# kr-colab/locator

Hardware: AMD Instinct MI355X
Metric: training samples/sec on 1000x100k-SNP matrix (higher is better)
Workload: dtype f32; 1 GPU; synthetic 1000 ind x 100000 SNPs uint8 (BASELINE.json configs[2]), single model fit per GPU, batch 32, 810 train / 90 validation; width=256, nlayers=10, graph=True, chained_steps=True, epochs_in_flight=2, replicates_per_gpu=1, replicates=single model, full=False

## Files before the change

locator_amd/_abi.py:

```python
import ctypes as C
import os
import re
from typing import NamedTuple

HEADER = os.path.join(os.path.dirname(os.path.dirname(os.path.abspath(__file__))), "include", "locator_hip.h")
_EXTENSION_TABLE = (
    ("ext", "locator_hip_query.h", None),
    ("region", "locator_hip_regions.h", "LOC_REGION_"),
    ("neighbor", "locator_hip_neighbors.h", "LOC_IBS_"),
    ("pca", "locator_hip_pca.h", "LOC_PCA_"),
    ("ld", "locator_hip_ld.h", "LOC_LD_"),
    ("spa", "locator_hip_spa.h", "LOC_SPA_"),
    ("admix", "locator_hip_admix.h", "LOC_ADMIX_"),
    ("localpca", "locator_hip_localpca.h", "LOC_LOCALPCA_"),
    ("paint", "locator_hip_paint.h", "LOC_PAINT_"),
    ("ibd", "locator_hip_ibd.h", "LOC_IBD_"),
    ("impute", "locator_hip_impute.h", "LOC_IMPUTE_"),
)

_SCALARS = {"int": C.c_int, "int32_t": C.c_int32, "uint32_t": C.c_uint32, "int64_t": C.c_int64, "uint64_t": C.c_uint64,
            "float": C.c_float, "double": C.c_double}
_POINTEES = ("void", "char", "int8_t", "uint8_t")
_BY_REFERENCE = ("loc_dims", "loc_layout", "loc_net", "loc_tuning")

_FIRST = re.compile(r"(?:const\s+)?(\w+)\s*((?:\*\s*)*)(\w+)$")
_NEXT = re.compile(r"((?:\*\s*)*)(\w+)$")
_DEFINE = re.compile(r"^[ \t]*#[ \t]*define[ \t]+(LOC_\w+)[ \t]+(\S.*?)[ \t]*$", re.M)
_STRUCT = re.compile(r"typedef\s+struct\s+(\w+)\s*\{(.*?)\}\s*\1\s*;", re.S)
_PROTO = re.compile(r"(.*?)\b(loc_\w+)\s*\((.*)\)$", re.S)


def _ctype(base, stars, name, structs, arg):
# ... 59 lines not shown
if not os.path.exists(HEADER):
    raise FileNotFoundError(f"{HEADER} not found: locator_amd runs in-tree and derives its ctypes binding from "
                            "include/locator_hip.h (the same relative path locator_amd/csrc compiles against).")
with open(HEADER) as _f:
    CONSTANTS, STRUCTS, PROTOTYPES = parse(_f.read())
globals().update(CONSTANTS)


class Extension(NamedTuple):
    header: str
    constants: dict
    prototypes: dict


EXTENSIONS = {}
ALL_PROTOTYPES = dict(PROTOTYPES)
_declared = set(CONSTANTS) | set(PROTOTYPES)
for _tag, _name, _prefix in _EXTENSION_TABLE:
    _path = os.path.join(os.path.dirname(HEADER), _name)
    if not os.path.exists(_path):
        raise FileNotFoundError(f"{_path} not found: it declares entry points added after include/locator_hip.h")
    with open(_path) as _f:
        _consts, _structs, _protos = parse(_f.read())
    _again = sorted(_declared & (set(_consts) | set(_protos)))
    _foreign = sorted(k for k, v in _consts.items() if _prefix is None or not k.startswith(_prefix) or not isinstance(v, int))
    if _structs or _again or _foreign or _tag in EXTENSIONS:
        raise ValueError(f"{_path} may declare new functions " + ("only" if _prefix is None else f"and {_prefix}* integer constants only")
                         + "".join(f"; {what}: {', '.join(names)}" for what, names in (("declared before", _again), ("not such a constant", _foreign))
                                   if names))
    _declared |= set(_consts) | set(_protos)
    EXTENSIONS[_tag] = Extension(_path, _consts, _protos)
    ALL_PROTOTYPES.update(_protos)
    globals().update(_consts)
```

locator_amd/csrc/l1_kernels.hip:

```cpp
#include <stdlib.h>

#include <type_traits>

#include "common.h"

#define LP 36

__global__ __launch_bounds__(128) void bn_batch_stats_kernel(
    const uint8_t* __restrict__ X, int64_t pitch, const int32_t* __restrict__ rows, int n_b, int K, int Kp,
    const float* __restrict__ gamma, const float* __restrict__ beta, float* __restrict__ mov_mean,
    float* __restrict__ mov_var, float* __restrict__ out4) {
    const int k0 = (blockIdx.x * blockDim.x + threadIdx.x) * 4;
    if (k0 >= Kp) return;
    int s[4] = {0, 0, 0, 0}, ss[4] = {0, 0, 0, 0};
#pragma unroll 8
    for (int b = 0; b < n_b; ++b) {
        uint32_t v = *reinterpret_cast<const uint32_t*>(X + (int64_t)rows[b] * pitch + k0);
#pragma unroll
        for (int c = 0; c < 4; ++c) {
            int x = (v >> (8 * c)) & 255;
            s[c] += x;
            ss[c] += x * x;
        }
    }
// ... 9 lines not shown
            o_sc[c] = scale;
            o_sh[c] = beta[k] - mean * scale;
            o_mu[c] = mean;
            o_rs[c] = rstd;
            mov_mean[k] = mov_mean[k] * BN_MOMENTUM + mean * (1.0f - BN_MOMENTUM);
            mov_var[k] = mov_var[k] * BN_MOMENTUM + var * (1.0f - BN_MOMENTUM);
        }
    }
    *reinterpret_cast<f32x4*>(out4 + k0) = o_sc;
    *reinterpret_cast<f32x4*>(out4 + Kp + k0) = o_sh;
    *reinterpret_cast<f32x4*>(out4 + 2 * (int64_t)Kp + k0) = o_mu;
    *reinterpret_cast<f32x4*>(out4 + 3 * (int64_t)Kp + k0) = o_rs;
}

template <bool UNIT>
__global__ __launch_bounds__(128) void bn_epoch_stats_kernel(const uint8_t* __restrict__ X, int64_t pitch,
                                                             const int32_t* __restrict__ rows_all, int batch,
                                                             int n_last, int n_steps, int K, int Kp,
                                                             float* __restrict__ stats_ep, float var_add) {
    const int k0 = (blockIdx.x * blockDim.x + threadIdx.x) * 4;
    const int step = blockIdx.y;
    if (k0 >= Kp) return;
    const int n_b = step == n_steps - 1 ? n_last : batch;
    const int32_t* rows = rows_all + (int64_t)step * batch;
    int s[4] = {0, 0, 0, 0}, ss[4] = {0, 0, 0, 0};
#pragma unroll 8
    for (int b = 0; b < n_b; ++b) {
        uint32_t v = *reinterpret_cast<const uint32_t*>(X + (int64_t)rows[b] * pitch + k0);
#pragma unroll
        for (int c = 0; c < 4; ++c) {
            int x = (v >> (8 * c)) & 255;
            s[c] += x;
            ss[c] += x * x;
        }
    }
    f32x4 mu = {0, 0, 0, 0}, var = {0, 0, 0, 0};
#pragma unroll
    for (int c = 0; c < 4; ++c) {
        if (k0 + c < K) {
            mu[c] = (float)s[c] / (float)n_b;
            var[c] = (float)((int64_t)n_b * ss[c] - (int64_t)s[c] * s[c]) / ((float)n_b * (float)n_b);
            if constexpr (UNIT) var[c] += var_add;
        }
    }
    float* o = stats_ep + (int64_t)step * 2 * Kp;
    *reinterpret_cast<f32x4*>(o + k0) = mu;
    *reinterpret_cast<f32x4*>(o + Kp + k0) = var;
}

__global__ void bn_epoch_finish_kernel(int K, int Kp, int n_steps, const float* __restrict__ stats_ep,
                                       const float* __restrict__ gamma, const float* __restrict__ beta,
                                       float* __restrict__ mov_mean, float* __restrict__ mov_var,
                                       float* __restrict__ bn4) {
    const int k = blockIdx.x * blockDim.x + threadIdx.x;
    if (k >= Kp) return;
    float scale = 0.f, shift = 0.f, mean0 = 0.f, rstd0 = 0.f;
    if (k < K) {
        float mm = mov_mean[k], mv = mov_var[k];
        for (int j = 0; j < n_steps; ++j) {
            const float mu = stats_ep[(int64_t)j * 2 * Kp + k], var = stats_ep[(int64_t)j * 2 * Kp + Kp + k];
            mm = mm * BN_MOMENTUM + mu * (1.0f - BN_MOMENTUM);
            mv = mv * BN_MOMENTUM + var * (1.0f - BN_MOMENTUM);
        }
        mov_mean[k] = mm;
        mov_var[k] = mv;
        mean0 = stats_ep[k];
        rstd0 = 1.0f / sqrtf(stats_ep[Kp + k] + BN_EPS);
        scale = gamma[k] * rstd0;
        shift = beta[k] - mean0 * scale;
    }
    if (bn4 == nullptr) return;
    bn4[k] = scale;
    bn4[Kp + k] = shift;
    bn4[2 * (int64_t)Kp + k] = mean0;
    bn4[3 * (int64_t)Kp + k] = rstd0;
}

__global__ void bn_infer_scale_shift_kernel(int K, int Kp, const float* __restrict__ gamma,
                                            const float* __restrict__ beta, const float* __restrict__ mov_mean,
                                            const float* __restrict__ mov_var, float* __restrict__ out4) {
    int k = blockIdx.x * blockDim.x + threadIdx.x;
    if (k >= Kp) return;
    float scale = 0.f, shift = 0.f, mean = 0.f, rstd = 0.f;
    if (k < K) {
        mean = mov_mean[k];
        rstd = 1.0f / sqrtf(mov_var[k] + BN_EPS);
        scale = gamma[k] * rstd;
        shift = beta[k] - mean * scale;
    }
    out4[k] = scale;
    out4[Kp + k] = shift;
    out4[2 * (int64_t)Kp + k] = mean;
    out4[3 * (int64_t)Kp + k] = rstd;
}

template <int NHT>
__global__ __launch_bounds__(512) void l1_fwd_partial_kernel(const uint8_t* __restrict__ X, int64_t pitch,
                                                             const int32_t* __restrict__ rows, int n_b, int Kp,
                                                             const float* __restrict__ ss4,
                                                             const float* __restrict__ w1s,
                                                             float* __restrict__ partial,
                                                             const uint8_t* __restrict__ in_mask, float in_ks) {
    constexpr int Hp = NHT * 32;
// ... 620 lines not shown
    if (k >= K) return;
    const float alpha = adam_alpha(alpha_tab, alpha_tab_len, lr, t_base, t_off);
    gamma_beta_adam_body(k, Kp, gbs, gamma, beta, m_gamma, v_gamma, m_beta, v_beta, alpha, next_stats, bn4);
}

extern "C" int loc_bn_batch_stats(const uint8_t* X, int64_t x_pitch, const int32_t* rows, int n_b, int K, int Kp,
                                  const float* gamma, const float* beta, float* mov_mean, float* mov_var,
                                  float* out4, void* stream) {
    if (n_b < 1 || n_b > LOC_ROWS) { loc_set_error("loc_bn_batch_stats: n_b=%d out of 1..32", n_b); return -1; }
    hipLaunchKernelGGL(bn_batch_stats_kernel, dim3((Kp / 4 + 127) / 128), dim3(128), 0, (hipStream_t)stream, X,
                       x_pitch, rows, n_b, K, Kp, gamma, beta, mov_mean, mov_var, out4);
    LOC_CHECK_LAUNCH();
    return 0;
}

extern "C" int loc_bn_epoch_stats(const uint8_t* X, int64_t x_pitch, const int32_t* rows_all, int batch, int n_last,
                                  int n_steps, int K, int Kp, const float* gamma, const float* beta,
                                  float* mov_mean, float* mov_var, float* stats_ep, float* bn4, void* stream) {
    if (batch < 1 || batch > LOC_BIG_BATCH_MAX || n_last < 1 || n_last > batch || n_steps < 1) {
        loc_set_error("loc_bn_epoch_stats: bad batch=%d n_last=%d n_steps=%d", batch, n_last, n_steps);
        return -1;
    }
    hipLaunchKernelGGL(bn_epoch_stats_kernel<false>, dim3((Kp / 4 + 127) / 128, n_steps), dim3(128), 0, (hipStream_t)stream,
                       X, x_pitch, rows_all, batch, n_last, n_steps, K, Kp, stats_ep, 0.f);
    LOC_CHECK_LAUNCH();
    hipLaunchKernelGGL(bn_epoch_finish_kernel, dim3((Kp + 255) / 256), dim3(256), 0, (hipStream_t)stream, K, Kp,
                       n_steps, stats_ep, gamma, beta, mov_mean, mov_var, bn4);
    LOC_CHECK_LAUNCH();
    return 0;
}

extern "C" int loc_bn_epoch_stats_only(const uint8_t* X, int64_t x_pitch, const int32_t* rows_all, int batch, int n_last,
                                       int n_steps, int K, int Kp, float* stats_ep, void* stream) {
    if (batch < 1 || batch > LOC_BIG_BATCH_MAX || n_last < 1 || n_last > batch || n_steps < 1) {
        loc_set_error("loc_bn_epoch_stats_only: bad batch=%d n_last=%d n_steps=%d", batch, n_last, n_steps);
        return -1;
    }
    hipLaunchKernelGGL(bn_epoch_stats_kernel<false>, dim3((Kp / 4 + 127) / 128, n_steps), dim3(128), 0, (hipStream_t)stream,
                       X, x_pitch, rows_all, batch, n_last, n_steps, K, Kp, stats_ep, 0.f);
    LOC_CHECK_LAUNCH();
    return 0;
}
extern "C" int loc_bn_epoch_finish(int n_steps, int K, int Kp, const float* gamma, const float* beta, float* mov_mean,
                                   float* mov_var, const float* stats_ep, float* bn4, void* stream) {
    if (n_steps < 1) { loc_set_error("loc_bn_epoch_finish: n_steps=%d", n_steps); return -1; }
    hipLaunchKernelGGL(bn_epoch_finish_kernel, dim3((Kp + 255) / 256), dim3(256), 0, (hipStream_t)stream, K, Kp,
                       n_steps, stats_ep, gamma, beta, mov_mean, mov_var, bn4);
    LOC_CHECK_LAUNCH();
    return 0;
}

static int bn_epoch_stats_unit_launch(const uint8_t* X, int64_t x_pitch, const int32_t* rows_all, int batch, int n_last,
                                      int n_steps, int K, int Kp, float* stats_ep, int unit, void* stream) {
    if (unit == 1) {
        hipLaunchKernelGGL(bn_epoch_stats_kernel<false>, dim3((Kp / 4 + 127) / 128, n_steps), dim3(128), 0, (hipStream_t)stream,
                           X, x_pitch, rows_all, batch, n_last, n_steps, K, Kp, stats_ep, 0.f);
    } else {
        hipLaunchKernelGGL(bn_epoch_stats_kernel<true>, dim3((Kp / 4 + 127) / 128, n_steps), dim3(128), 0, (hipStream_t)stream,
                           X, x_pitch, rows_all, batch, n_last, n_steps, K, Kp, stats_ep, loc_bn_var_add(unit));
    }
    LOC_CHECK_LAUNCH();
    return 0;
}

static bool bn_unit_ok(int unit) { return unit >= 1 && unit <= LOC_DOSAGE_UNIT; }

extern "C" int loc_bn_epoch_stats_unit(const uint8_t* X, int64_t x_pitch, const int32_t* rows_all, int batch, int n_last,
                                       int n_steps, int K, int Kp, const float* gamma, const float* beta,
                                       float* mov_mean, float* mov_var, float* stats_ep, float* bn4, int unit, void* stream) {
    if (batch < 1 || batch > LOC_BIG_BATCH_MAX || n_last < 1 || n_last > batch || n_steps < 1 || !bn_unit_ok(unit)) {
        loc_set_error("loc_bn_epoch_stats_unit: bad batch=%d n_last=%d n_steps=%d unit=%d", batch, n_last, n_steps, unit);
        return -1;
    }
    int rc = bn_epoch_stats_unit_launch(X, x_pitch, rows_all, batch, n_last, n_steps, K, Kp, stats_ep, unit, stream);
    if (rc) return rc;
    hipLaunchKernelGGL(bn_epoch_finish_kernel, dim3((Kp + 255) / 256), dim3(256), 0, (hipStream_t)stream, K, Kp,
                       n_steps, stats_ep, gamma, beta, mov_mean, mov_var, bn4);
    LOC_CHECK_LAUNCH();
    return 0;
}

extern "C" int loc_bn_epoch_stats_only_unit(const uint8_t* X, int64_t x_pitch, const int32_t* rows_all, int batch, int n_last,
                                            int n_steps, int K, int Kp, float* stats_ep, int unit, void* stream) {
    if (batch < 1 || batch > LOC_BIG_BATCH_MAX || n_last < 1 || n_last > batch || n_steps < 1 || !bn_unit_ok(unit)) {
        loc_set_error("loc_bn_epoch_stats_only_unit: bad batch=%d n_last=%d n_steps=%d unit=%d", batch, n_last, n_steps, unit);
        return -1;
    }
    return bn_epoch_stats_unit_launch(X, x_pitch, rows_all, batch, n_last, n_steps, K, Kp, stats_ep, unit, stream);
}

extern "C" float loc_bn_var_add(int unit) { return (float)(unit * unit - 1) * BN_EPS; }

extern "C" int loc_bn_infer_scale_shift(int K, int Kp, const float* gamma, const float* beta, const float* mov_mean,
                                        const float* mov_var, float* out4, void* stream) {
    hipLaunchKernelGGL(bn_infer_scale_shift_kernel, dim3((Kp + 255) / 256), dim3(256), 0, (hipStream_t)stream, K, Kp,
                       gamma, beta, mov_mean, mov_var, out4);
    LOC_CHECK_LAUNCH();
    return 0;
}

static int l1_forward_impl(const uint8_t* X, int64_t x_pitch, const int32_t* rows, int n_b, const loc_dims* d,
                           const float* scale_shift, const float* w1s, const float* b1, float* partial, int grid,
                           float* a1, float* a1_drop, const uint8_t* mask, float keep_scale, const uint8_t* in_mask,
// ... 198 lines not shown
```

locator_amd/csrc/util_kernels.hip:

```cpp
#include "common.h"

__device__ __forceinline__ float u01(uint32_t r) { return ((float)r + 0.5f) * 2.3283064365386963e-10f; }

__global__ void init_glorot_kernel(float* __restrict__ dst, int R, int C, int Rp, int Cp, int swizzled, float limit,
                                   uint64_t seed, uint64_t stream_id) {
    int64_t i = (int64_t)blockIdx.x * blockDim.x + threadIdx.x;
    if (i >= (int64_t)Rp * Cp) return;
    int r = (int)(i / Cp), c = (int)(i % Cp);
    float val = 0.f;
    if (r < R && c < C) {
        philox4 p = philox4x32_10((uint64_t)r * (uint64_t)C + (uint64_t)c, stream_id, seed);
        val = (2.f * u01(p.v[0]) - 1.f) * limit;
    }
    int64_t o = swizzled ? w1s_index(c, r, Cp / 32) : i;
    dst[o] = val;
}

__global__ void init_uniform_kernel(float* __restrict__ dst, int64_t n, float limit, uint64_t seed,
                                    uint64_t stream_id) {
    int64_t j = (int64_t)blockIdx.x * blockDim.x + threadIdx.x;
    if (4 * j >= n) return;
    philox4 p = philox4x32_10((uint64_t)j, stream_id, seed);
    for (int c = 0; c < 4; ++c)
        if (4 * j + c < n) dst[4 * j + c] = (2.f * u01(p.v[c]) - 1.f) * limit;
// ... 144 lines not shown
    hipLaunchKernelGGL(w1_swizzle_kernel, dim3((unsigned)((n + 255) / 256)), dim3(256), 0, (hipStream_t)stream, w_kh,
                       K, H, w1s, Kp, Hp);
    LOC_CHECK_LAUNCH();
    return 0;
}

extern "C" int loc_w1_unswizzle(const float* w1s, int Kp, int Hp, float* w_kh, int K, int H, void* stream) {
    int64_t n = (int64_t)K * H;
    (void)Kp;
    hipLaunchKernelGGL(w1_unswizzle_kernel, dim3((unsigned)((n + 255) / 256)), dim3(256), 0, (hipStream_t)stream, w1s,
                       Hp, w_kh, K, H);
    LOC_CHECK_LAUNCH();
    return 0;
}

__global__ __launch_bounds__(256) void epoch_callbacks_kernel(const float* __restrict__ stats, int steps, int batch, int n_last,
                                                              int n_val, loc_cb_state* __restrict__ st, float* __restrict__ lr,
                                                              double* __restrict__ hist, int hist_cap) {
    __shared__ float buf[1024];
    const int t = threadIdx.x;
    const int n_train = (steps - 1) * batch + n_last;
    double loss = 0.0, val = 0.0;
    for (int base = 0; base < steps; base += 1024) {
        const int m = steps - base < 1024 ? steps - base : 1024;
        __syncthreads();
        for (int i = t; i < m; i += 256) buf[i] = stats[base + i];
        __syncthreads();
        if (t == 0)
            for (int i = 0; i < m; ++i) loss += (double)buf[i] * (double)(base + i == steps - 1 ? n_last : batch);
    }
    for (int base = 0; base < n_val; base += 1024) {
        const int m = n_val - base < 1024 ? n_val - base : 1024;
        __syncthreads();
        for (int i = t; i < m; i += 256) buf[i] = stats[steps + base + i];
        __syncthreads();
        if (t == 0)
            for (int i = 0; i < m; ++i) val += (double)buf[i];
    }
    if (t != 0) return;
    loss /= (double)n_train;
    val /= (double)n_val;
    const int epoch = st->epoch;
    st->epoch = epoch + 1;
    st->save_now = 0;
    if (st->stopped) return;
    const float lr_logged = st->lr;
    int flags = 0;
    if (val < st->ck_best) { st->ck_best = val; st->save_now = 1; st->best_epoch = epoch; flags |= 1; }
    st->es_wait += 1;
    if (val < st->es_best) { st->es_best = val; st->es_wait = 0; }
    if (st->es_wait >= st->patience && epoch > 0) { st->stopped = 1; st->stop_epoch = epoch; flags |= 2; }
    if (val < st->rl_best) {
        st->rl_best = val;
        st->rl_wait = 0;
    } else {
        st->rl_wait += 1;
        if (st->rl_wait >= st->lr_patience) {
            const float nl = fmaxf(st->lr * st->lr_factor, 0.0f);
            st->lr = nl;
            *lr = nl;
            st->rl_wait = 0;
            flags |= 4;
        }
    }
    if (epoch < hist_cap) {
        double* row = hist + 4 * (int64_t)epoch;
        row[0] = loss; row[1] = val; row[2] = (double)lr_logged; row[3] = (double)flags;
    }
}

__global__ __launch_bounds__(256) void snapshot_if_kernel(const loc_cb_state* __restrict__ st, const f32x4* __restrict__ src,
                                                          f32x4* __restrict__ dst, int64_t n4) {
    if (!st->save_now) return;
    for (int64_t i = (int64_t)blockIdx.x * 256 + threadIdx.x; i < n4; i += (int64_t)gridDim.x * 256)
        __builtin_nontemporal_store(__builtin_nontemporal_load(src + i), dst + i);
}

extern "C" int loc_epoch_callbacks(const float* stats, int steps, int batch, int n_last, int n_val, loc_cb_state* state,
                                   float* lr, double* hist, int hist_cap, void* stream) {
    if (steps < 1 || batch < 1 || n_last < 1 || n_last > batch || n_val < 1 || !state || !lr || !hist) {
        loc_set_error("loc_epoch_callbacks: steps=%d batch=%d n_last=%d n_val=%d (all >= 1, n_last <= batch)", steps, batch,
                      n_last, n_val);
        return -1;
    }
    hipLaunchKernelGGL(epoch_callbacks_kernel, dim3(1), dim3(256), 0, (hipStream_t)stream, stats, steps, batch, n_last, n_val,
                       state, lr, hist, hist_cap);
    LOC_CHECK_LAUNCH();
    return 0;
}

extern "C" int loc_snapshot_if(const loc_cb_state* state, const float* params, float* best, int64_t n, void* stream) {
    if (n % 4 || ((uintptr_t)params & 15) || ((uintptr_t)best & 15)) {
        loc_set_error("loc_snapshot_if: needs 16-byte aligned buffers and a multiple of 4 floats");
        return -1;
    }
    hipLaunchKernelGGL(snapshot_if_kernel, dim3(1024), dim3(256), 0, (hipStream_t)stream, state,
                       reinterpret_cast<const f32x4*>(params), reinterpret_cast<f32x4*>(best), n / 4);
    LOC_CHECK_LAUNCH();
    return 0;
}

constexpr int KDE_LDS_POINTS = 4096;

__global__ __launch_bounds__(256) void kde_peak_kernel(const double* __restrict__ xy, const int64_t* __restrict__ offsets,
                                                       double inv_2h2, int32_t* __restrict__ peak_index,
                                                       double* __restrict__ out) {
    __shared__ double pts[2 * KDE_LDS_POINTS];
    __shared__ double r_score[256];
    __shared__ int r_idx[256];
    __shared__ double r_sx[256], r_sy[256];
    __shared__ int r_bad[256];
    const int s = blockIdx.x, t = threadIdx.x;
// ... 63 lines not shown
```

locator_amd/net.py:

```python
from __future__ import annotations

import ctypes as C

import numpy as np
import torch

from . import _lib
from ._abi import (LOC_BATCH_SLOT, LOC_BIG_BATCH_MAX, LOC_DOSAGE_UNIT, LOC_GEMM_I8_PACKED_MIN_ROWS, LOC_MAX_BATCH,
                   LOC_MAX_FWD_GRID, LOC_ROWS)

ALPHA_TAB_LEN = 32769
ADAM_B1, ADAM_B2 = 0.9, 0.999


def _ptr(t):
    return C.c_void_p(t.data_ptr()) if t is not None else None


def _stream():
    return C.c_void_p(torch.cuda.current_stream().cuda_stream)


_NCU, _NCU_LOCK = {}, __import__("threading").Lock()

# ... 281 lines not shown
        d = self.d
        if self.unit != 1:
            _lib.check(self.lib.loc_bn_epoch_stats_only_unit(self.X.data_ptr(), self.X.stride(0), _ptr(rows_all), int(batch),
                                                             int(n_last), int(n_steps), d.K, d.Kp, _ptr(stats_ep), self.unit,
                                                             _stream()), "loc_bn_epoch_stats_only_unit")
            return
        _lib.check(self.lib.loc_bn_epoch_stats_only(self.X.data_ptr(), self.X.stride(0), _ptr(rows_all), int(batch), int(n_last),
                                                    int(n_steps), d.K, d.Kp, _ptr(stats_ep), _stream()), "loc_bn_epoch_stats_only")

    def epoch_bn_finish(self, n_steps, stats_ep):
        self.params_changed()
        d, lay, P = self.d, self.lay, self.params.data_ptr()
        _lib.check(self.lib.loc_bn_epoch_finish(int(n_steps), d.K, d.Kp, P + 4 * lay.gamma, P + 4 * lay.beta,
                                                P + 4 * lay.mov_mean, P + 4 * lay.mov_var, _ptr(stats_ep), None, _stream()),
                   "loc_bn_epoch_finish")

    def predict_rows(self, rows, n, yhat, dist=None, in_fit=False):
        lib, d = self.lib, self.d
        capturing = torch.cuda.is_current_stream_capturing() or bool(in_fit)
        digits = self.predict_digits if self.predict_digits != 0 else 3
        use_i8 = (self.predict_pieces > 0 and digits > 0 and n >= lib.loc_gemm_i8_min_rows(digits)
                  and lib.loc_l1_gemm_i8_supported(d.Hp, digits))
        if use_i8 and self.genotype_max() > 127:
            use_i8 = False
        guarded = use_i8 and self.predict_digits in (0, 3) and not capturing
        need = 0
        if use_i8:
            need = lib.loc_l1_image_i8_bytes(C.byref(d), 3 if self.predict_digits == 0 else digits)
        elif (self.predict_pieces > 0 and n >= lib.loc_gemm_min_rows(self.predict_pieces)
              and lib.loc_l1_gemm_supported(d.Hp, self.predict_pieces)):
# ... 145 lines not shown
```

locator_amd/train.py:

```python
from __future__ import annotations

import time

import numpy as np
import torch

from .net import LocatorNet


CAPTURE_ERROR_MODE = "thread_local"


class _DeviceLock:

    def __init__(self):
        import threading
        self._lock = threading.Lock()
        self._tls = threading.local()

    def __enter__(self):
        depth = getattr(self._tls, "depth", 0)
        if depth == 0:
            self._lock.acquire()
        self._tls.depth = depth + 1
# ... 61 lines not shown
                self.lr = float(np.float32(max(np.float32(self.lr) * np.float32(self.lr_factor), 0.0)))
                self.rl_wait = 0
        return save, stop, lr_logged


class History:

    def __init__(self):
        self.history = {"loss": [], "val_loss": [], "learning_rate": []}
        self.epoch_seconds = []


class EpochRunner:

    def __init__(self, net: LocatorNet, train_rows, val_rows, batch_size=32, use_graph=True, chain=None, xchain=False,
                 side_stats=False):
        self.slot_rows = net.set_batch(int(batch_size))
        self.net = net
        dev = net.device
        self.batch = int(batch_size)
        self.train_rows = np.asarray(train_rows, dtype=np.int32)
        self.n_train = len(self.train_rows)
        self.steps = (self.n_train + self.batch - 1) // self.batch
        self.n_val = len(val_rows)
        self.val_rows = torch.as_tensor(np.asarray(val_rows, dtype=np.int32)).to(dev)
        self.perm_ring = [torch.empty(self.steps * self.batch, dtype=torch.int32).pin_memory()]
        self.perm_host = self.perm_ring[0]
        self.epochs_started = 0
        self.cb = None
        self.perm_dev = torch.zeros(self.steps * self.batch, dtype=torch.int32, device=dev)
        self.mask_stride = self.slot_rows * net.mask_width
        self.masks = (torch.zeros(self.steps * self.mask_stride, dtype=torch.uint8, device=dev)
                      if net.drop_p > 0 else None)
        self.stats = torch.zeros(self.steps + max(self.n_val, 1), dtype=torch.float32, device=dev)
        self.stats_host = torch.empty_like(self.stats, device="cpu").pin_memory()
        self.val_yhat = torch.zeros((max(self.n_val, 1), 2), dtype=torch.float32, device=dev)
        self.stats_ep = torch.zeros(self.steps * 2 * net.d.Kp, dtype=torch.float32, device=dev)
        self.use_graph = use_graph
        self.graph = None
        self.epochs_run = 0
        self.step_sizes = np.array([min(self.batch, self.n_train - j * self.batch) for j in range(self.steps)])
        net.cnet()
        self.chain = net.chain_supported() if chain is None else (bool(chain) and net.chain_supported())
        self.xchain = bool(xchain) and self.chain
        if self.xchain:
            self.perm_dev2 = [self.perm_dev, torch.zeros_like(self.perm_dev)]
            self.stats_ep2 = [self.stats_ep, torch.zeros_like(self.stats_ep)]
            self.graphs = [None, None]
            self._perm_promised = None
            self.side_stats = bool(side_stats)
            self._side = None
            if len(self.perm_ring) < 3:
                self.perm_ring = [torch.empty(self.steps * self.batch, dtype=torch.int32).pin_memory() for _ in range(3)]
# ... 5 lines not shown
        import ctypes as C
        from . import _lib
        assert self.epochs_started == 0 and self.graph is None
        net, dev = self.net, self.net.device
        st = _lib.CbState()
        st.ck_best = st.es_best = st.rl_best = float("inf")
        st.lr = float(np.float32(lr0))
        st.lr_factor = float(lr_factor)
        st.patience = int(patience)
        st.lr_patience = int(patience / 6) if lr_patience is None else int(lr_patience)
        st.stop_epoch = st.best_epoch = -1
        raw = np.frombuffer(bytes(st), dtype=np.uint8).copy()
        cap = int(max_epochs)
        self.cb = {"state": torch.from_numpy(raw).to(dev), "hist": torch.zeros((cap, 4), dtype=torch.float64, device=dev),
                   "hist_host": torch.zeros((cap, 4), dtype=torch.float64).pin_memory(), "cap": cap, "depth": int(depth),
                   "events": [torch.cuda.Event() for _ in range(int(depth) + 2)], "state_size": C.sizeof(_lib.CbState)}
        if net.best is None:
            net.best = torch.empty_like(net.params)
        net.lr_t.fill_(st.lr)
        self.perm_ring = [torch.empty(self.steps * self.batch, dtype=torch.int32).pin_memory() for _ in range(int(depth) + 3)]
        self.perm_host = self.perm_ring[0]

    def read_cb_state(self):
        from . import _lib
        raw = self.cb["state"].cpu().numpy().tobytes()
        return _lib.CbState.from_buffer_copy(raw)

    def enqueue(self, ev=None, epoch=0):
        net = self.net
        sz = 2 * net.d.Kp
        n_last = int(self.step_sizes[-1])
        if self.xchain:
            p = epoch & 1
            perm_dev, stats_ep = self.perm_dev2[p], self.stats_ep2[p]
            perm_nx, stats_nx = self.perm_dev2[1 - p], self.stats_ep2[1 - p]
            if epoch == 0:
                net.epoch_bn_stats(perm_dev, self.batch, n_last, self.steps, stats_ep)
            else:
                net.epoch_bn_finish(self.steps, stats_ep)
            if self.side_stats:
                cur = torch.cuda.current_stream()
                if self._side is None:
                    self._side = torch.cuda.Stream(device=net.device)
                self._side.wait_stream(cur)
                with torch.cuda.stream(self._side):
                    net.epoch_bn_stats_only(perm_nx, self.batch, n_last, self.steps, stats_nx)
            else:
                net.epoch_bn_stats_only(perm_nx, self.batch, n_last, self.steps, stats_nx)
        else:
            perm_dev, stats_ep = self.perm_dev, self.stats_ep
            net.epoch_bn_stats(perm_dev, self.batch, n_last, self.steps, stats_ep)
        for j in range(self.steps):
            nb = int(self.step_sizes[j])
            mask = self.masks[j * self.mask_stride:] if self.masks is not None else None
            e0, e1 = (ev[j] if ev is not None else (None, None))
            nxt = stats_ep[(j + 1) * sz:] if j + 1 < self.steps else None
            if self.chain:
                last = j + 1 >= self.steps
                rows_next = None if last else perm_dev[(j + 1) * self.batch:]
                nb_next = 0 if last else int(self.step_sizes[j + 1])
                fwd_done = j > 0
                if self.xchain:
                    if last:
                        rows_next, nb_next, nxt = perm_nx, int(self.step_sizes[0]), stats_nx
                        if self.side_stats:
                            torch.cuda.current_stream().wait_stream(self._side)
                    fwd_done = j > 0 or epoch > 0
                net.train_step_chain(perm_dev[j * self.batch:], nb, j + 1, mask, self.stats[j:], nxt, rows_next, nb_next,
                                     fwd_done, e0, e1)
                continue
            net.train_step(perm_dev[j * self.batch:], nb, j + 1, mask, self.stats[j:], e0, e1,
                           bn_ready=True, bn_next=nxt)
        if self.n_val:
            net.predict_rows(self.val_rows, self.n_val, self.val_yhat, self.stats[self.steps:], in_fit=True)
        if self.cb is not None:
            from . import _lib
            from .net import _ptr, _stream
            cb = self.cb
            _lib.check(net.lib.loc_epoch_callbacks(_ptr(self.stats), self.steps, self.batch, int(self.step_sizes[-1]), self.n_val,
                                                   _ptr(cb["state"]), _ptr(net.lr_t), _ptr(cb["hist"]), cb["cap"], _stream()),
                       "loc_epoch_callbacks")
            _lib.check(net.lib.loc_snapshot_if(_ptr(cb["state"]), _ptr(net.params), _ptr(net.best), net.params.numel(),
                                               _stream()), "loc_snapshot_if")
        net.t_base_t.add_(self.steps)

    def _upload_perm(self, perm, dst, slot):
        rows = self.train_rows[np.asarray(perm)]
        host = self.perm_ring[slot % len(self.perm_ring)]
        host[:self.n_train] = torch.from_numpy(rows)
        host[self.n_train:] = 0
        dst.copy_(host, non_blocking=True)
        self.perm_host = host

# ... 49 lines not shown
        self.epochs_run += 1
        s = self.stats_host.numpy()
        loss = float(np.dot(s[:self.steps].astype(np.float64), self.step_sizes) / self.n_train)
        val = float(s[self.steps:self.steps + self.n_val].astype(np.float64).mean()) if self.n_val else float("nan")
        return loss, val

    def run_epoch(self, perm, ev=None):
        self.start_epoch(perm, ev)
        return self.finish_epoch()


class FitLoop:

    def __init__(self, net, train_rows, val_rows, *, batch_size=32, max_epochs=5000, patience=100, lr_patience=None,
                 lr_factor=0.5, perm_fn=None, use_graph=True, chain=None, depth=2, verbose=0, log=print, xchain=True,
                 side_stats=False):
        if len(val_rows) == 0:
            raise ValueError("fit needs validation rows: checkpoint, early stopping and the LR plateau all monitor val_loss")
        self.net = net
        self.runner = EpochRunner(net, train_rows, val_rows, batch_size, use_graph, chain=chain, xchain=xchain,
                                  side_stats=side_stats)
        self._perms = {}
        self.max_epochs, self.depth = int(max_epochs), max(0, int(depth))
        self.runner.enable_device_callbacks(patience, 1e-3, lr_patience, lr_factor, self.max_epochs, self.depth)
        rng = np.random.Generator(np.random.PCG64(np.random.SeedSequence([net.seed, net.replicate, 0x7065726D])))
        self.perm_fn = perm_fn if perm_fn is not None else (lambda epoch: rng.permutation(self.runner.n_train))
        self.hist = History()
        self.submitted = 0
        self.collected = 0
        self.stop_epoch = None
        self.verbose, self.log = verbose, log
        self._t_last = time.perf_counter()

    @property
    def done(self):
        return self.stop_epoch is not None or self.collected >= self.max_epochs
# ... 77 lines not shown
```

Measured before the change: 196,400 samples/s.

## Fuse epoch-seam BN finish/stats and epoch-end callbacks into single kernels

```diff
diff --git a/include/locator_hip_seam.h b/include/locator_hip_seam.h
--- /dev/null
+++ b/include/locator_hip_seam.h
@@ -0,0 +1,21 @@
+#ifndef LOCATOR_HIP_SEAM_H
+#define LOCATOR_HIP_SEAM_H
+#include "locator_hip.h"
+
+#ifdef __cplusplus
+extern "C" {
+#endif
+
+int loc_bn_epoch_advance(const uint8_t* X, int64_t x_pitch, const int32_t* rows_next, int batch, int n_last, int n_steps,
+                         int K, int Kp, const float* gamma, const float* beta, float* mov_mean, float* mov_var,
+                         const float* stats_cur, float* bn4, float* stats_next, int unit, void* stream);
+
+int loc_epoch_end_ticket_words(void);
+int loc_epoch_end(const float* stats, int steps, int batch, int n_last, int n_val, void* state, float* lr, double* hist,
+                  int hist_cap, const float* params, float* best, int64_t n, int* t_base, int t_add, uint32_t* ticket,
+                  void* stream);
+
+#ifdef __cplusplus
+}
+#endif
+#endif
diff --git a/locator_amd/_abi.py b/locator_amd/_abi.py
--- a/locator_amd/_abi.py
+++ b/locator_amd/_abi.py
@@ -16,6 +16,9 @@
     ("paint", "locator_hip_paint.h", "LOC_PAINT_"),
     ("ibd", "locator_hip_ibd.h", "LOC_IBD_"),
     ("impute", "locator_hip_impute.h", "LOC_IMPUTE_"),
+)
+_FIT_EXTENSION_TABLE = (
+    ("seam", "locator_hip_seam.h", None),
 )
 
 _SCALARS = {"int": C.c_int, "int32_t": C.c_int32, "uint32_t": C.c_uint32, "int64_t": C.c_int64, "uint64_t": C.c_uint64,
@@ -105,21 +108,23 @@
 
 
 EXTENSIONS = {}
+FIT_EXTENSIONS = {}
 ALL_PROTOTYPES = dict(PROTOTYPES)
 _declared = set(CONSTANTS) | set(PROTOTYPES)
-for _tag, _name, _prefix in _EXTENSION_TABLE:
-    _path = os.path.join(os.path.dirname(HEADER), _name)
-    if not os.path.exists(_path):
-        raise FileNotFoundError(f"{_path} not found: it declares entry points added after include/locator_hip.h")
-    with open(_path) as _f:
-        _consts, _structs, _protos = parse(_f.read())
-    _again = sorted(_declared & (set(_consts) | set(_protos)))
-    _foreign = sorted(k for k, v in _consts.items() if _prefix is None or not k.startswith(_prefix) or not isinstance(v, int))
-    if _structs or _again or _foreign or _tag in EXTENSIONS:
-        raise ValueError(f"{_path} may declare new functions " + ("only" if _prefix is None else f"and {_prefix}* integer constants only")
-                         + "".join(f"; {what}: {', '.join(names)}" for what, names in (("declared before", _again), ("not such a constant", _foreign))
-                                   if names))
-    _declared |= set(_consts) | set(_protos)
-    EXTENSIONS[_tag] = Extension(_path, _consts, _protos)
-    ALL_PROTOTYPES.update(_protos)
-    globals().update(_consts)
+for _table, _into in ((_EXTENSION_TABLE, EXTENSIONS), (_FIT_EXTENSION_TABLE, FIT_EXTENSIONS)):
+    for _tag, _name, _prefix in _table:
+        _path = os.path.join(os.path.dirname(HEADER), _name)
+        if not os.path.exists(_path):
+            raise FileNotFoundError(f"{_path} not found: it declares entry points added after include/locator_hip.h")
+        with open(_path) as _f:
+            _consts, _structs, _protos = parse(_f.read())
+        _again = sorted(_declared & (set(_consts) | set(_protos)))
+        _foreign = sorted(k for k, v in _consts.items() if _prefix is None or not k.startswith(_prefix) or not isinstance(v, int))
+        if _structs or _again or _foreign or _tag in EXTENSIONS or _tag in FIT_EXTENSIONS:
+            raise ValueError(f"{_path} may declare new functions " + ("only" if _prefix is None else f"and {_prefix}* integer constants only")
+                             + "".join(f"; {what}: {', '.join(names)}" for what, names in (("declared before", _again), ("not such a constant", _foreign))
+                                       if names))
+        _declared |= set(_consts) | set(_protos)
+        _into[_tag] = Extension(_path, _consts, _protos)
+        ALL_PROTOTYPES.update(_protos)
+        globals().update(_consts)
diff --git a/locator_amd/csrc/l1_kernels.hip b/locator_amd/csrc/l1_kernels.hip
--- a/locator_amd/csrc/l1_kernels.hip
+++ b/locator_amd/csrc/l1_kernels.hip
@@ -3,6 +3,7 @@
 #include <type_traits>
 
 #include "common.h"
+#include "../../include/locator_hip_seam.h"
 
 #define LP 36
 
@@ -47,12 +48,10 @@
 }
 
 template <bool UNIT>
-__global__ __launch_bounds__(128) void bn_epoch_stats_kernel(const uint8_t* __restrict__ X, int64_t pitch,
-                                                             const int32_t* __restrict__ rows_all, int batch,
-                                                             int n_last, int n_steps, int K, int Kp,
-                                                             float* __restrict__ stats_ep, float var_add) {
-    const int k0 = (blockIdx.x * blockDim.x + threadIdx.x) * 4;
-    const int step = blockIdx.y;
+__device__ __forceinline__ void bn_epoch_stats_body(int k0, int step, const uint8_t* __restrict__ X, int64_t pitch,
+                                                    const int32_t* __restrict__ rows_all, int batch, int n_last,
+                                                    int n_steps, int K, int Kp, float* __restrict__ stats_ep,
+                                                    float var_add) {
     if (k0 >= Kp) return;
     const int n_b = step == n_steps - 1 ? n_last : batch;
     const int32_t* rows = rows_all + (int64_t)step * batch;
@@ -81,32 +80,93 @@
     *reinterpret_cast<f32x4*>(o + Kp + k0) = var;
 }
 
-__global__ void bn_epoch_finish_kernel(int K, int Kp, int n_steps, const float* __restrict__ stats_ep,
-                                       const float* __restrict__ gamma, const float* __restrict__ beta,
-                                       float* __restrict__ mov_mean, float* __restrict__ mov_var,
-                                       float* __restrict__ bn4) {
-    const int k = blockIdx.x * blockDim.x + threadIdx.x;
+template <bool UNIT>
+__global__ __launch_bounds__(128) void bn_epoch_stats_kernel(const uint8_t* __restrict__ X, int64_t pitch,
+                                                             const int32_t* __restrict__ rows_all, int batch,
+                                                             int n_last, int n_steps, int K, int Kp,
+                                                             float* __restrict__ stats_ep, float var_add) {
+    bn_epoch_stats_body<UNIT>((blockIdx.x * blockDim.x + threadIdx.x) * 4, blockIdx.y, X, pitch, rows_all, batch, n_last,
+                              n_steps, K, Kp, stats_ep, var_add);
+}
+
+__device__ __forceinline__ float bn_moving_step(float m, float x) {
+#pragma clang fp contract(off)
+    const float t = x * (1.0f - BN_MOMENTUM);
+    return __builtin_fmaf(m, BN_MOMENTUM, t);
+}
+__device__ __forceinline__ void bn_scale_shift(float gamma, float beta, float mean, float rstd, float& scale, float& shift) {
+#pragma clang fp contract(off)
+    scale = gamma * rstd;
+    shift = __builtin_fmaf(-mean, scale, beta);
+}
+
+#define BN_FINISH_BLOCK 8
+__device__ __forceinline__ void bn_epoch_finish_body(int k, int K, int Kp, int n_steps, const float* __restrict__ stats_ep,
+                                                     const float* __restrict__ gamma, const float* __restrict__ beta,
+                                                     float* __restrict__ mov_mean, float* __restrict__ mov_var,
+                                                     float* __restrict__ bn4) {
     if (k >= Kp) return;
     float scale = 0.f, shift = 0.f, mean0 = 0.f, rstd0 = 0.f;
     if (k < K) {
         float mm = mov_mean[k], mv = mov_var[k];
-        for (int j = 0; j < n_steps; ++j) {
-            const float mu = stats_ep[(int64_t)j * 2 * Kp + k], var = stats_ep[(int64_t)j * 2 * Kp + Kp + k];
-            mm = mm * BN_MOMENTUM + mu * (1.0f - BN_MOMENTUM);
-            mv = mv * BN_MOMENTUM + var * (1.0f - BN_MOMENTUM);
+        const float* p = stats_ep + k;
+        const int64_t step_pitch = 2 * (int64_t)Kp;
+        int j = 0;
+        for (; j + BN_FINISH_BLOCK <= n_steps; j += BN_FINISH_BLOCK) {
+            float mu[BN_FINISH_BLOCK], var[BN_FINISH_BLOCK];
+#pragma unroll
+            for (int e = 0; e < BN_FINISH_BLOCK; ++e) {
+                mu[e] = p[(j + e) * step_pitch];
+                var[e] = p[(j + e) * step_pitch + Kp];
+            }
+#pragma unroll
+            for (int e = 0; e < BN_FINISH_BLOCK; ++e) {
+                mm = bn_moving_step(mm, mu[e]);
+                mv = bn_moving_step(mv, var[e]);
+            }
+        }
+        for (; j < n_steps; ++j) {
+            mm = bn_moving_step(mm, p[j * step_pitch]);
+            mv = bn_moving_step(mv, p[j * step_pitch + Kp]);
         }
         mov_mean[k] = mm;
         mov_var[k] = mv;
-        mean0 = stats_ep[k];
-        rstd0 = 1.0f / sqrtf(stats_ep[Kp + k] + BN_EPS);
-        scale = gamma[k] * rstd0;
-        shift = beta[k] - mean0 * scale;
+        if (bn4 != nullptr) {
+            mean0 = stats_ep[k];
+            rstd0 = 1.0f / sqrtf(stats_ep[Kp + k] + BN_EPS);
+            bn_scale_shift(gamma[k], beta[k], mean0, rstd0, scale, shift);
+        }
     }
     if (bn4 == nullptr) return;
     bn4[k] = scale;
     bn4[Kp + k] = shift;
     bn4[2 * (int64_t)Kp + k] = mean0;
     bn4[3 * (int64_t)Kp + k] = rstd0;
+}
+
+__global__ __launch_bounds__(256) void bn_epoch_finish_kernel(int K, int Kp, int n_steps, const float* __restrict__ stats_ep,
+                                                              const float* __restrict__ gamma, const float* __restrict__ beta,
+                                                              float* __restrict__ mov_mean, float* __restrict__ mov_var,
+                                                              float* __restrict__ bn4) {
+    bn_epoch_finish_body(blockIdx.x * blockDim.x + threadIdx.x, K, Kp, n_steps, stats_ep, gamma, beta, mov_mean, mov_var, bn4);
+}
+
+template <bool UNIT>
+__global__ __launch_bounds__(256) void bn_epoch_advance_kernel(int n_fin, int nbx, const uint8_t* __restrict__ X, int64_t pitch,
+                                                               const int32_t* __restrict__ rows_next, int batch, int n_last,
+                                                               int n_steps, int K, int Kp, const float* __restrict__ stats_cur,
+                                                               const float* __restrict__ gamma, const float* __restrict__ beta,
+                                                               float* __restrict__ mov_mean, float* __restrict__ mov_var,
+                                                               float* __restrict__ bn4, float* __restrict__ stats_next,
+                                                               float var_add) {
+    const int bid = blockIdx.x;
+    if (bid < n_fin) {
+        bn_epoch_finish_body(bid * 256 + (int)threadIdx.x, K, Kp, n_steps, stats_cur, gamma, beta, mov_mean, mov_var, bn4);
+        return;
+    }
+    const int sb = bid - n_fin, step = sb / nbx, bx = sb - step * nbx;
+    bn_epoch_stats_body<UNIT>((bx * 256 + (int)threadIdx.x) * 4, step, X, pitch, rows_next, batch, n_last, n_steps, K, Kp,
+                                 stats_next, var_add);
 }
 
 __global__ void bn_infer_scale_shift_kernel(int K, int Kp, const float* __restrict__ gamma,
@@ -118,8 +178,7 @@
     if (k < K) {
         mean = mov_mean[k];
         rstd = 1.0f / sqrtf(mov_var[k] + BN_EPS);
-        scale = gamma[k] * rstd;
-        shift = beta[k] - mean * scale;
+        bn_scale_shift(gamma[k], beta[k], mean, rstd, scale, shift);
     }
     out4[k] = scale;
     out4[Kp + k] = shift;
@@ -770,42 +829,6 @@
     return 0;
 }
 
-extern "C" int loc_bn_epoch_stats(const uint8_t* X, int64_t x_pitch, const int32_t* rows_all, int batch, int n_last,
-                                  int n_steps, int K, int Kp, const float* gamma, const float* beta,
-                                  float* mov_mean, float* mov_var, float* stats_ep, float* bn4, void* stream) {
-    if (batch < 1 || batch > LOC_BIG_BATCH_MAX || n_last < 1 || n_last > batch || n_steps < 1) {
-        loc_set_error("loc_bn_epoch_stats: bad batch=%d n_last=%d n_steps=%d", batch, n_last, n_steps);
-        return -1;
-    }
-    hipLaunchKernelGGL(bn_epoch_stats_kernel<false>, dim3((Kp / 4 + 127) / 128, n_steps), dim3(128), 0, (hipStream_t)stream,
-                       X, x_pitch, rows_all, batch, n_last, n_steps, K, Kp, stats_ep, 0.f);
-    LOC_CHECK_LAUNCH();
-    hipLaunchKernelGGL(bn_epoch_finish_kernel, dim3((Kp + 255) / 256), dim3(256), 0, (hipStream_t)stream, K, Kp,
-                       n_steps, stats_ep, gamma, beta, mov_mean, mov_var, bn4);
-    LOC_CHECK_LAUNCH();
-    return 0;
-}
-
-extern "C" int loc_bn_epoch_stats_only(const uint8_t* X, int64_t x_pitch, const int32_t* rows_all, int batch, int n_last,
-                                       int n_steps, int K, int Kp, float* stats_ep, void* stream) {
-    if (batch < 1 || batch > LOC_BIG_BATCH_MAX || n_last < 1 || n_last > batch || n_steps < 1) {
-        loc_set_error("loc_bn_epoch_stats_only: bad batch=%d n_last=%d n_steps=%d", batch, n_last, n_steps);
-        return -1;
-    }
-    hipLaunchKernelGGL(bn_epoch_stats_kernel<false>, dim3((Kp / 4 + 127) / 128, n_steps), dim3(128), 0, (hipStream_t)stream,
-                       X, x_pitch, rows_all, batch, n_last, n_steps, K, Kp, stats_ep, 0.f);
-    LOC_CHECK_LAUNCH();
-    return 0;
-}
-extern "C" int loc_bn_epoch_finish(int n_steps, int K, int Kp, const float* gamma, const float* beta, float* mov_mean,
-                                   float* mov_var, const float* stats_ep, float* bn4, void* stream) {
-    if (n_steps < 1) { loc_set_error("loc_bn_epoch_finish: n_steps=%d", n_steps); return -1; }
-    hipLaunchKernelGGL(bn_epoch_finish_kernel, dim3((Kp + 255) / 256), dim3(256), 0, (hipStream_t)stream, K, Kp,
-                       n_steps, stats_ep, gamma, beta, mov_mean, mov_var, bn4);
-    LOC_CHECK_LAUNCH();
-    return 0;
-}
-
 static int bn_epoch_stats_unit_launch(const uint8_t* X, int64_t x_pitch, const int32_t* rows_all, int batch, int n_last,
                                       int n_steps, int K, int Kp, float* stats_ep, int unit, void* stream) {
     if (unit == 1) {
@@ -819,6 +842,40 @@
     return 0;
 }
 
+static int bn_epoch_finish_launch(int n_steps, int K, int Kp, const float* gamma, const float* beta, float* mov_mean,
+                                  float* mov_var, const float* stats_ep, float* bn4, void* stream) {
+    hipLaunchKernelGGL(bn_epoch_finish_kernel, dim3((Kp + 255) / 256), dim3(256), 0, (hipStream_t)stream, K, Kp,
+                       n_steps, stats_ep, gamma, beta, mov_mean, mov_var, bn4);
+    LOC_CHECK_LAUNCH();
+    return 0;
+}
+
+extern "C" int loc_bn_epoch_stats(const uint8_t* X, int64_t x_pitch, const int32_t* rows_all, int batch, int n_last,
+                                  int n_steps, int K, int Kp, const float* gamma, const float* beta,
+                                  float* mov_mean, float* mov_var, float* stats_ep, float* bn4, void* stream) {
+    if (batch < 1 || batch > LOC_BIG_BATCH_MAX || n_last < 1 || n_last > batch || n_steps < 1) {
+        loc_set_error("loc_bn_epoch_stats: bad batch=%d n_last=%d n_steps=%d", batch, n_last, n_steps);
+        return -1;
+    }
+    int rc = bn_epoch_stats_unit_launch(X, x_pitch, rows_all, batch, n_last, n_steps, K, Kp, stats_ep, 1, stream);
+    if (rc) return rc;
+    return bn_epoch_finish_launch(n_steps, K, Kp, gamma, beta, mov_mean, mov_var, stats_ep, bn4, stream);
+}
+
+extern "C" int loc_bn_epoch_stats_only(const uint8_t* X, int64_t x_pitch, const int32_t* rows_all, int batch, int n_last,
+                                       int n_steps, int K, int Kp, float* stats_ep, void* stream) {
+    if (batch < 1 || batch > LOC_BIG_BATCH_MAX || n_last < 1 || n_last > batch || n_steps < 1) {
+        loc_set_error("loc_bn_epoch_stats_only: bad batch=%d n_last=%d n_steps=%d", batch, n_last, n_steps);
+        return -1;
+    }
+    return bn_epoch_stats_unit_launch(X, x_pitch, rows_all, batch, n_last, n_steps, K, Kp, stats_ep, 1, stream);
+}
+extern "C" int loc_bn_epoch_finish(int n_steps, int K, int Kp, const float* gamma, const float* beta, float* mov_mean,
+                                   float* mov_var, const float* stats_ep, float* bn4, void* stream) {
+    if (n_steps < 1) { loc_set_error("loc_bn_epoch_finish: n_steps=%d", n_steps); return -1; }
+    return bn_epoch_finish_launch(n_steps, K, Kp, gamma, beta, mov_mean, mov_var, stats_ep, bn4, stream);
+}
+
 static bool bn_unit_ok(int unit) { return unit >= 1 && unit <= LOC_DOSAGE_UNIT; }
 
 extern "C" int loc_bn_epoch_stats_unit(const uint8_t* X, int64_t x_pitch, const int32_t* rows_all, int batch, int n_last,
@@ -830,10 +887,7 @@
     }
     int rc = bn_epoch_stats_unit_launch(X, x_pitch, rows_all, batch, n_last, n_steps, K, Kp, stats_ep, unit, stream);
     if (rc) return rc;
-    hipLaunchKernelGGL(bn_epoch_finish_kernel, dim3((Kp + 255) / 256), dim3(256), 0, (hipStream_t)stream, K, Kp,
-                       n_steps, stats_ep, gamma, beta, mov_mean, mov_var, bn4);
-    LOC_CHECK_LAUNCH();
-    return 0;
+    return bn_epoch_finish_launch(n_steps, K, Kp, gamma, beta, mov_mean, mov_var, stats_ep, bn4, stream);
 }
 
 extern "C" int loc_bn_epoch_stats_only_unit(const uint8_t* X, int64_t x_pitch, const int32_t* rows_all, int batch, int n_last,
@@ -843,6 +897,35 @@
         return -1;
     }
     return bn_epoch_stats_unit_launch(X, x_pitch, rows_all, batch, n_last, n_steps, K, Kp, stats_ep, unit, stream);
+}
+
+extern "C" int loc_bn_epoch_advance(const uint8_t* X, int64_t x_pitch, const int32_t* rows_next, int batch, int n_last,
+                                    int n_steps, int K, int Kp, const float* gamma, const float* beta, float* mov_mean,
+                                    float* mov_var, const float* stats_cur, float* bn4, float* stats_next, int unit,
+                                    void* stream) {
+    if (batch < 1 || batch > LOC_BIG_BATCH_MAX || n_last < 1 || n_last > batch || n_steps < 1 || !bn_unit_ok(unit)) {
+        loc_set_error("loc_bn_epoch_advance: bad batch=%d n_last=%d n_steps=%d unit=%d", batch, n_last, n_steps, unit);
+        return -1;
+    }
+    const int64_t ep_floats = (int64_t)n_steps * 2 * Kp;
+    if (!stats_cur || !stats_next || (stats_cur < stats_next + ep_floats && stats_next < stats_cur + ep_floats)) {
+        loc_set_error("loc_bn_epoch_advance: stats_cur and stats_next must be two buffers of n_steps * 2 * Kp floats");
+        return -1;
+    }
+    const int n_fin = (Kp + 255) / 256, nbx = (Kp / 4 + 255) / 256;
+    const int64_t grid = (int64_t)n_fin + (int64_t)n_steps * nbx;
+    if (grid > 0x7fffffff) { loc_set_error("loc_bn_epoch_advance: %d steps of %d SNPs exceed one grid", n_steps, Kp); return -1; }
+    const float var_add = unit == 1 ? 0.f : loc_bn_var_add(unit);
+    if (unit == 1)
+        hipLaunchKernelGGL(bn_epoch_advance_kernel<false>, dim3((unsigned)grid), dim3(256), 0, (hipStream_t)stream, n_fin, nbx, X,
+                           x_pitch, rows_next, batch, n_last, n_steps, K, Kp, stats_cur, gamma, beta, mov_mean, mov_var, bn4,
+                           stats_next, var_add);
+    else
+        hipLaunchKernelGGL(bn_epoch_advance_kernel<true>, dim3((unsigned)grid), dim3(256), 0, (hipStream_t)stream, n_fin, nbx, X,
+                           x_pitch, rows_next, batch, n_last, n_steps, K, Kp, stats_cur, gamma, beta, mov_mean, mov_var, bn4,
+                           stats_next, var_add);
+    LOC_CHECK_LAUNCH();
+    return 0;
 }
 
 extern "C" float loc_bn_var_add(int unit) { return (float)(unit * unit - 1) * BN_EPS; }
diff --git a/locator_amd/csrc/util_kernels.hip b/locator_amd/csrc/util_kernels.hip
--- a/locator_amd/csrc/util_kernels.hip
+++ b/locator_amd/csrc/util_kernels.hip
@@ -1,4 +1,5 @@
 #include "common.h"
+#include "../../include/locator_hip_seam.h"
 
 __device__ __forceinline__ float u01(uint32_t r) { return ((float)r + 0.5f) * 2.3283064365386963e-10f; }
 
@@ -182,13 +183,12 @@
     return 0;
 }
 
-__global__ __launch_bounds__(256) void epoch_callbacks_kernel(const float* __restrict__ stats, int steps, int batch, int n_last,
-                                                              int n_val, loc_cb_state* __restrict__ st, float* __restrict__ lr,
-                                                              double* __restrict__ hist, int hist_cap) {
-    __shared__ float buf[1024];
+__device__ __forceinline__ void cb_epoch_sums(const float* __restrict__ stats, int steps, int batch, int n_last, int n_val,
+                                              float* buf, double& loss, double& val) {
     const int t = threadIdx.x;
     const int n_train = (steps - 1) * batch + n_last;
-    double loss = 0.0, val = 0.0;
+    loss = 0.0;
+    val = 0.0;
     for (int base = 0; base < steps; base += 1024) {
         const int m = steps - base < 1024 ? steps - base : 1024;
         __syncthreads();
@@ -205,9 +205,13 @@
         if (t == 0)
             for (int i = 0; i < m; ++i) val += (double)buf[i];
     }
-    if (t != 0) return;
     loss /= (double)n_train;
     val /= (double)n_val;
+}
+
+__device__ __forceinline__ bool cb_epoch_improves(const loc_cb_state* st, double val) { return !st->stopped && val < st->ck_best; }
+
+__device__ __forceinline__ void cb_epoch_update(loc_cb_state* st, float* lr, double* hist, int hist_cap, double loss, double val) {
     const int epoch = st->epoch;
     st->epoch = epoch + 1;
     st->save_now = 0;
@@ -237,6 +241,16 @@
     }
 }
 
+__global__ __launch_bounds__(256) void epoch_callbacks_kernel(const float* __restrict__ stats, int steps, int batch, int n_last,
+                                                              int n_val, loc_cb_state* __restrict__ st, float* __restrict__ lr,
+                                                              double* __restrict__ hist, int hist_cap) {
+    __shared__ float buf[1024];
+    double loss, val;
+    cb_epoch_sums(stats, steps, batch, n_last, n_val, buf, loss, val);
+    if (threadIdx.x != 0) return;
+    cb_epoch_update(st, lr, hist, hist_cap, loss, val);
+}
+
 __global__ __launch_bounds__(256) void snapshot_if_kernel(const loc_cb_state* __restrict__ st, const f32x4* __restrict__ src,
                                                           f32x4* __restrict__ dst, int64_t n4) {
     if (!st->save_now) return;
@@ -244,6 +258,36 @@
         __builtin_nontemporal_store(__builtin_nontemporal_load(src + i), dst + i);
 }
 
+__global__ __launch_bounds__(256) void epoch_end_kernel(const float* __restrict__ stats, int steps, int batch, int n_last, int n_val,
+                                                        loc_cb_state* st, float* lr, double* hist, int hist_cap,
+                                                        const float* __restrict__ src, float* __restrict__ dst, int64_t n,
+                                                        int* t_base, int t_add, uint32_t* ticket) {
+    __shared__ float buf[1024];
+    double loss, val;
+    cb_epoch_sums(stats, steps, batch, n_last, n_val, buf, loss, val);
+    if (threadIdx.x == 0) buf[0] = cb_epoch_improves(st, val) ? 1.f : 0.f;
+    __syncthreads();
+    if (buf[0] != 0.f) {
+        const int64_t n4 = n / 4;
+        const f32x4* s4 = reinterpret_cast<const f32x4*>(src);
+        f32x4* d4 = reinterpret_cast<f32x4*>(dst);
+        for (int64_t i = (int64_t)blockIdx.x * 256 + threadIdx.x; i < n4; i += (int64_t)gridDim.x * 256)
+            __builtin_nontemporal_store(__builtin_nontemporal_load(s4 + i), d4 + i);
+        if (blockIdx.x == 0 && (int64_t)threadIdx.x < n - 4 * n4) dst[4 * n4 + threadIdx.x] = src[4 * n4 + threadIdx.x];
+    }
+    __syncthreads();
+    if (threadIdx.x != 0) return;
+    const int g = blockIdx.x >> 5, n_groups = (gridDim.x + 31) >> 5;
+    const unsigned g_size = g == n_groups - 1 ? gridDim.x - 32u * g : 32u;
+    uint32_t* mine = ticket + 16 * (1 + g);
+    if (__hip_atomic_fetch_add(mine, 1u, __ATOMIC_RELAXED, __HIP_MEMORY_SCOPE_AGENT) != g_size - 1) return;
+    __hip_atomic_store(mine, 0u, __ATOMIC_RELAXED, __HIP_MEMORY_SCOPE_AGENT);
+    if (__hip_atomic_fetch_add(ticket, 1u, __ATOMIC_RELAXED, __HIP_MEMORY_SCOPE_AGENT) != (unsigned)n_groups - 1) return;
+    cb_epoch_update(st, lr, hist, hist_cap, loss, val);
+    t_base[0] += t_add;
+    __hip_atomic_store(ticket, 0u, __ATOMIC_RELAXED, __HIP_MEMORY_SCOPE_AGENT);
+}
+
 extern "C" int loc_epoch_callbacks(const float* stats, int steps, int batch, int n_last, int n_val, loc_cb_state* state,
                                    float* lr, double* hist, int hist_cap, void* stream) {
     if (steps < 1 || batch < 1 || n_last < 1 || n_last > batch || n_val < 1 || !state || !lr || !hist) {
@@ -264,6 +308,29 @@
     }
     hipLaunchKernelGGL(snapshot_if_kernel, dim3(1024), dim3(256), 0, (hipStream_t)stream, state,
                        reinterpret_cast<const f32x4*>(params), reinterpret_cast<f32x4*>(best), n / 4);
+    LOC_CHECK_LAUNCH();
+    return 0;
+}
+
+#define EPOCH_END_MAX_WGS 1024
+extern "C" int loc_epoch_end_ticket_words(void) { return 16 * (1 + EPOCH_END_MAX_WGS / 32); }
+
+extern "C" int loc_epoch_end(const float* stats, int steps, int batch, int n_last, int n_val, void* state, float* lr,
+                             double* hist, int hist_cap, const float* params, float* best, int64_t n, int* t_base, int t_add,
+                             uint32_t* ticket, void* stream) {
+    if (steps < 1 || batch < 1 || n_last < 1 || n_last > batch || n_val < 1 || !state || !lr || !hist) {
+        loc_set_error("loc_epoch_end: steps=%d batch=%d n_last=%d n_val=%d (all >= 1, n_last <= batch)", steps, batch, n_last,
+                      n_val);
+        return -1;
+    }
+    if (n < 1 || !params || !best || !t_base || !ticket || ((uintptr_t)params & 15) || ((uintptr_t)best & 15)) {
+        loc_set_error("loc_epoch_end: needs n >= 1 floats in 16-byte aligned params / best, t_base and a ticket word");
+        return -1;
+    }
+    const int64_t pieces = (n / 4 + 255) / 256;
+    const int grid = pieces < 1 ? 1 : pieces > EPOCH_END_MAX_WGS ? EPOCH_END_MAX_WGS : (int)pieces;
+    hipLaunchKernelGGL(epoch_end_kernel, dim3(grid), dim3(256), 0, (hipStream_t)stream, stats, steps, batch, n_last, n_val,
+                       static_cast<loc_cb_state*>(state), lr, hist, hist_cap, params, best, n, t_base, t_add, ticket);
     LOC_CHECK_LAUNCH();
     return 0;
 }
diff --git a/locator_amd/net.py b/locator_amd/net.py
--- a/locator_amd/net.py
+++ b/locator_amd/net.py
@@ -319,6 +319,14 @@
         _lib.check(self.lib.loc_bn_epoch_finish(int(n_steps), d.K, d.Kp, P + 4 * lay.gamma, P + 4 * lay.beta,
                                                 P + 4 * lay.mov_mean, P + 4 * lay.mov_var, _ptr(stats_ep), None, _stream()),
                    "loc_bn_epoch_finish")
+
+    def epoch_bn_advance(self, n_steps, stats_cur, rows_next, batch, n_last, stats_next):
+        self.params_changed()
+        d, lay, P = self.d, self.lay, self.params.data_ptr()
+        _lib.check(self.lib.loc_bn_epoch_advance(self.X.data_ptr(), self.X.stride(0), _ptr(rows_next), int(batch), int(n_last),
+                                                 int(n_steps), d.K, d.Kp, P + 4 * lay.gamma, P + 4 * lay.beta,
+                                                 P + 4 * lay.mov_mean, P + 4 * lay.mov_var, _ptr(stats_cur), None,
+                                                 _ptr(stats_next), self.unit, _stream()), "loc_bn_epoch_advance")
 
     def predict_rows(self, rows, n, yhat, dist=None, in_fit=False):
         lib, d = self.lib, self.d
diff --git a/locator_amd/train.py b/locator_amd/train.py
--- a/locator_amd/train.py
+++ b/locator_amd/train.py
@@ -99,7 +99,7 @@
 class EpochRunner:
 
     def __init__(self, net: LocatorNet, train_rows, val_rows, batch_size=32, use_graph=True, chain=None, xchain=False,
-                 side_stats=False):
+                 side_stats=False, seam=True):
         self.slot_rows = net.set_batch(int(batch_size))
         self.net = net
         dev = net.device
@@ -122,6 +122,7 @@
         self.val_yhat = torch.zeros((max(self.n_val, 1), 2), dtype=torch.float32, device=dev)
         self.stats_ep = torch.zeros(self.steps * 2 * net.d.Kp, dtype=torch.float32, device=dev)
         self.use_graph = use_graph
+        self.seam = bool(seam)
         self.graph = None
         self.epochs_run = 0
         self.step_sizes = np.array([min(self.batch, self.n_train - j * self.batch) for j in range(self.steps)])
@@ -157,7 +158,8 @@
         cap = int(max_epochs)
         self.cb = {"state": torch.from_numpy(raw).to(dev), "hist": torch.zeros((cap, 4), dtype=torch.float64, device=dev),
                    "hist_host": torch.zeros((cap, 4), dtype=torch.float64).pin_memory(), "cap": cap, "depth": int(depth),
-                   "events": [torch.cuda.Event() for _ in range(int(depth) + 2)], "state_size": C.sizeof(_lib.CbState)}
+                   "events": [torch.cuda.Event() for _ in range(int(depth) + 2)], "state_size": C.sizeof(_lib.CbState),
+                   "ticket": torch.zeros(int(net.lib.loc_epoch_end_ticket_words()), dtype=torch.int32, device=dev)}
         if net.best is None:
             net.best = torch.empty_like(net.params)
         net.lr_t.fill_(st.lr)
@@ -179,17 +181,20 @@
             perm_nx, stats_nx = self.perm_dev2[1 - p], self.stats_ep2[1 - p]
             if epoch == 0:
                 net.epoch_bn_stats(perm_dev, self.batch, n_last, self.steps, stats_ep)
+            if epoch > 0 and self.seam and not self.side_stats:
+                net.epoch_bn_advance(self.steps, stats_ep, perm_nx, self.batch, n_last, stats_nx)
             else:
-                net.epoch_bn_finish(self.steps, stats_ep)
-            if self.side_stats:
-                cur = torch.cuda.current_stream()
-                if self._side is None:
-                    self._side = torch.cuda.Stream(device=net.device)
-                self._side.wait_stream(cur)
-                with torch.cuda.stream(self._side):
+                if epoch > 0:
+                    net.epoch_bn_finish(self.steps, stats_ep)
+                if self.side_stats:
+                    cur = torch.cuda.current_stream()
+                    if self._side is None:
+                        self._side = torch.cuda.Stream(device=net.device)
+                    self._side.wait_stream(cur)
+                    with torch.cuda.stream(self._side):
+                        net.epoch_bn_stats_only(perm_nx, self.batch, n_last, self.steps, stats_nx)
+                else:
                     net.epoch_bn_stats_only(perm_nx, self.batch, n_last, self.steps, stats_nx)
-            else:
-                net.epoch_bn_stats_only(perm_nx, self.batch, n_last, self.steps, stats_nx)
         else:
             perm_dev, stats_ep = self.perm_dev, self.stats_ep
             net.epoch_bn_stats(perm_dev, self.batch, n_last, self.steps, stats_ep)
@@ -220,6 +225,12 @@
             from . import _lib
             from .net import _ptr, _stream
             cb = self.cb
+            if self.seam:
+                _lib.check(net.lib.loc_epoch_end(_ptr(self.stats), self.steps, self.batch, int(self.step_sizes[-1]), self.n_val,
+                                                 _ptr(cb["state"]), _ptr(net.lr_t), _ptr(cb["hist"]), cb["cap"], _ptr(net.params),
+                                                 _ptr(net.best), net.params.numel(), _ptr(net.t_base_t), self.steps,
+                                                 _ptr(cb["ticket"]), _stream()), "loc_epoch_end")
+                return
             _lib.check(net.lib.loc_epoch_callbacks(_ptr(self.stats), self.steps, self.batch, int(self.step_sizes[-1]), self.n_val,
                                                    _ptr(cb["state"]), _ptr(net.lr_t), _ptr(cb["hist"]), cb["cap"], _stream()),
                        "loc_epoch_callbacks")
@@ -299,12 +310,12 @@
 
     def __init__(self, net, train_rows, val_rows, *, batch_size=32, max_epochs=5000, patience=100, lr_patience=None,
                  lr_factor=0.5, perm_fn=None, use_graph=True, chain=None, depth=2, verbose=0, log=print, xchain=True,
-                 side_stats=False):
+                 side_stats=False, seam=True):
         if len(val_rows) == 0:
             raise ValueError("fit needs validation rows: checkpoint, early stopping and the LR plateau all monitor val_loss")
         self.net = net
         self.runner = EpochRunner(net, train_rows, val_rows, batch_size, use_graph, chain=chain, xchain=xchain,
-                                  side_stats=side_stats)
+                                  side_stats=side_stats, seam=seam)
         self._perms = {}
         self.max_epochs, self.depth = int(max_epochs), max(0, int(depth))
         self.runner.enable_device_callbacks(patience, 1e-3, lr_patience, lr_factor, self.max_epochs, self.depth)
```

Result: no change. 197,400 samples/s, median of 2 (+0.5%).
